# multigrid101/Opt

Measured on AMD Instinct MI355X. Metric: PCG JᵀJ·p throughput (unknowns/s) + GN iters/s, image_warping 4096² fp32, higher is better.
Workload: dtype f32; 1 GPU; image_warping 4096x4096 fp32 GN+PCG, lIterations=10; unknowns=50331648, parallelism=single

## Files before the change

opt_amd/csrc/common.h:

```cpp
#pragma once
#include <hip/hip_runtime.h>
#include <cstdio>
#include <cstdlib>
#include <cstdint>

#define OPT_HIP_CHECK(call)                                                         \
    do {                                                                            \
        hipError_t e_ = (call);                                                     \
        if (e_ != hipSuccess) {                                                     \
            fprintf(stderr, "[opt_amd] HIP error %d (%s) in %s at %s:%d\n", (int)e_,\
                    hipGetErrorString(e_), #call, __FILE__, __LINE__);              \
            exit(1);                                                                \
        }                                                                           \
    } while (0)

namespace optamd {

#define OPTAMD_HAVE_KBLOCK
constexpr int kWave = 64;
constexpr int kBlock = 256;
constexpr int kMaxReduce = 4;

struct Domain {
    int W, H;
    int y_lo, y_hi;
    int y_mem0, mem_rows;
    int edges = 0;
    __host__ __device__ long long npix_mem() const { return (long long)W * mem_rows; }
    __host__ __device__ long long off(int x, int yg) const {
        return (long long)(yg - y_mem0) * W + x;
    }
};

struct VecLayout {
    int nimg;
    int ch[4];
    long long off[5];
    long long N;
    long long fbase[4];
    __host__ __device__ static long long div_ch(long long l, int c) {
        switch (c) {
            case 1: return l;
            case 2: return l >> 1;
            case 3: return l < (1LL << 32) ? (long long)((unsigned)l / 3u) : l / 3;
            case 4: return l >> 2;
            default: return l / c;
        }
    }
    __host__ __device__ long long locate(long long e, int* img, long long* local) const {
        int k = 0;
        while (k + 1 < nimg && e >= off[k + 1]) ++k;
        *img = k;
        *local = e - off[k];
        return fbase[k] + div_ch(*local, ch[k]);
// ... 99 lines not shown
```

opt_amd/csrc/image_warping.hip:

```cpp
#include <hip/hip_runtime.h>
#include <hip/hip_ext.h>
#include <algorithm>
#include <type_traits>
#include <cmath>
#include <cstring>
#include <string>
#include "plan.h"
#include "pcg_kernels.h"
#include "stencil_plan.h"

namespace optamd {
namespace iw {
#pragma clang fp contract(on)

constexpr int kStrip = 64;

inline int rows_for(int nstrips, int nrows) {
    int rows = 32;
    while (rows > 16 && (long long)nstrips * ((nrows + 4 * rows - 1) / (4 * rows)) < 2048) rows /= 2;
    return rows;
}
inline int rows_one_round(int ngroups, int nrows, int ncu) {
    const long long slots = 4LL * 4 * ncu;
    for (int r = 8; r < 16; ++r)
        if ((long long)ngroups * ((nrows + r - 1) / r) * 4 <= slots) return r;
    return 16;
}

template <typename T>
struct Args {
    Domain dom;
    const T* O;
    const T* A;
    const float* U;
    const float* C;
    const float* M;
    uint8_t* flags;
    T wf, wr;
    int use_pre;
    int nstrips, nrowblocks, rows;
    int tb0, tn0, tb1;
    int side;
    int rev;
    T* S;
    T preO[2][5];
};

__shared__ float iw_ptab_f[16];
__shared__ double iw_ptab_d[16];
template <typename T> __device__ __forceinline__ T* iw_ptab();
template <> __device__ __forceinline__ float* iw_ptab<float>() { return iw_ptab_f; }
template <> __device__ __forceinline__ double* iw_ptab<double>() { return iw_ptab_d; }

template <typename T>
__device__ __forceinline__ T pre_offset(const Args<T>&, int f) {
    return (f & 1) ? iw_ptab<T>()[(f >> 1) & 15] : (T)0;
}
template <typename T>
__device__ __forceinline__ T pre_entry(const Args<T>& a, int k) {
    return k < 10 ? a.preO[k & 1][k >> 1] : (T)0;
}
#define IW_PRE_TABLE(a)                                                           \
    if (threadIdx.x < 16) iw_ptab<T>()[threadIdx.x] = pre_entry(a, threadIdx.x); \
    __syncthreads();

template <bool NT, typename T>
__device__ __forceinline__ T ld_v(const T* p) {
    if constexpr (NT) return __builtin_nontemporal_load(p);
    else return *p;
}
template <bool NT, typename T>
__device__ __forceinline__ void st_v(T* p, T v) {
    if constexpr (NT) __builtin_nontemporal_store(v, p);
    else *p = v;
}

// ... 42 lines not shown
__device__ __forceinline__ bool present(const Domain& d, int x, int y) {
    return x >= 0 && x < d.W && y >= 0 && y < d.H && y >= d.y_mem0 && y < d.y_mem0 + d.mem_rows;
}

template <typename T>
__device__ __forceinline__ void jedge(T pjx, T pjy, T pjt, T cj, T sj, float ujx, float ujy,
                                      T ptx, T pty, float utx, float uty, bool v, T wr,
                                      T& Jx, T& Jy, T& ax, T& ay) {
    const T dx = (T)(ujx - utx), dy = (T)(ujy - uty);
    ax = -sj * dx - cj * dy;
    ay = cj * dx - sj * dy;
    Jx = v ? wr * (pjx - ptx - ax * pjt) : (T)0;
    Jy = v ? wr * (pjy - pty - ay * pjt) : (T)0;
}

template <typename T>
__device__ __forceinline__ void eedge(T ojx, T ojy, T cj, T sj, float ujx, float ujy, T otx,
                                      T oty, float utx, float uty, bool v, T wr, T& ex, T& ey,
                                      T& ax, T& ay) {
    const T dx = (T)(ujx - utx), dy = (T)(ujy - uty);
    const T rx = cj * dx - sj * dy, ry = sj * dx + cj * dy;
    ax = -sj * dx - cj * dy;
    ay = cj * dx - sj * dy;
    ex = v ? wr * (ojx - otx - rx) : (T)0;
    ey = v ? wr * (ojy - oty - ry) : (T)0;
}

template <typename T>
__device__ __forceinline__ T diag_a2(T cj, T sj, float ujx, float ujy, float utx, float uty, T wr2) {
    const T dx = (T)(ujx - utx), dy = (T)(ujy - uty);
    const T ax = fmad(-sj, dx, -opaque(cj * dy));
    const T ay = fmad(cj, dx, -opaque(sj * dy));
    return opaque(wr2 * fmad(ax, ax, opaque(ay * ay)));
}

template <typename T>
__device__ __forceinline__ T pre_angle(T dt) {
    const T st = (T)1 + sqrt(dt);
    return (T)1 / (st * st);
}

typedef double acc_t;
template <typename T>
__device__ __forceinline__ T pcg_alpha(double rz, double pap) {
    return pap > 0.0 ? (T)(rz / pap) : (T)0;
}
template <typename T>
__device__ __forceinline__ acc_t dot3(T a0, T b0, T a1, T b1, T a2, T b2) {
    return (double)a0 * (double)b0 + (double)a1 * (double)b1 + (double)a2 * (double)b2;
}
template <typename T>
__device__ __forceinline__ acc_t wdot3(T w0, T a0, T b0, T w1, T a1, T b1, T w2, T a2, T b2) {
    (void)w1;
    return (double)w0 * ((double)a0 * (double)b0 + (double)a1 * (double)b1) + (double)w2 * ((double)a2 * (double)b2);
}

template <typename T>
struct PRaw {
    T v0, v1, v2;
    T w0, w1, w2;
    T q0, q1, q2;
    T d0, d1, d2;
    T ang;
    float2 u;
    int f, in;
    T ev0, ev1, ev2, ew0, ew1, ew2, eq0, eq1, eq2, eang;
// ... 480 lines not shown
                rapd += wdot3(cur.w0, cur.rx, aox, cur.w0, cur.ry, aoy, cur.w2, cur.rt, aot);
                apapd += wdot3(cur.w0, aox, aox, cur.w0, aoy, aoy, cur.w2, aot, aot);
            }
            in_up_x = jpy_x; in_up_y = jpy_y;
            my_x = jdn_x; my_y = jdn_y;
            thm = -wr * (adn_x * jdn_x + adn_y * jdn_y);
        };
        for (int y = g.y0; y < g.y1; y += 2) {
            const RRaw<T> n1 = raw(min(y + 2, g.y1));
            apply_row(A, B, y);
            A = fin(n1, y + 2);
            if (y + 1 >= g.y1) break;
            const RRaw<T> n2 = raw(min(y + 3, g.y1));
            apply_row(B, A, y + 1);
            B = fin(n2, y + 3);
        }
    }
    double v[4] = {(double)rzd, (double)papd, (double)rapd, (double)apapd};
    block_reduce_publish<4>(v, rs, g.tile);
}

template <typename T>
__device__ __forceinline__ vec2_t<T> shl2(vec2_t<T> v) {
    vec2_t<T> o;
    o.x = from_left0(v.x); o.y = from_left0(v.y);
    return o;
}
template <typename T>
__device__ __forceinline__ vec2_t<T> shr2(vec2_t<T> v) {
    vec2_t<T> o;
    o.x = from_right0(v.x); o.y = from_right0(v.y);
    return o;
}
template <typename T>
__device__ __forceinline__ void jedge2(vec2_t<T> pj, T pjt, T cj, T sj, vec2_t<float> uj, vec2_t<T> pt,
                                       vec2_t<float> ut, bool v, T wr, vec2_t<T>& J, vec2_t<T>& ad) {
    const vec2_t<float> du = uj - ut;
    const T dx = (T)du.x, dy = (T)du.y;
    vec2_t<T> ms, cs;
    ms.x = -sj; ms.y = cj;
    cs.x = cj; cs.y = sj;
    ad = ms * dx - cs * dy;
    const vec2_t<T> j = wr * ((pj - pt) - ad * pjt);
    J = v ? j : (vec2_t<T>)0;
}
template <typename T>
struct ACarry {
    vec2_t<T> in_up, my;
    T thm;
};
template <typename T>
__device__ __forceinline__ ACarry<T> acarry_init(vec2_t<T> up, T upt, T uc, T us, vec2_t<float> uu, bool uact,
                                                 vec2_t<T> cp, T cpt, T cc, T cs, vec2_t<float> cu, bool cact, T wr) {
    ACarry<T> k;
    vec2_t<T> ad;
    jedge2(up, upt, uc, us, uu, cp, cu, uact && cact, wr, k.in_up, ad);
    jedge2(cp, cpt, cc, cs, cu, up, uu, uact && cact, wr, k.my, ad);
    const vec2_t<T> th = ad * k.my;
    k.thm = -wr * (th.x + th.y);
    return k;
}
template <typename T>
__device__ __forceinline__ void apply_ap2(vec2_t<T> cp, T cpt, T cc, T cs, vec2_t<float> cu, bool cact, bool cfit,
                                          vec2_t<T> dp, T dpt, T dc, T ds, vec2_t<float> du, bool dact, T wr, T wf2,
                                          ACarry<T>& k, vec2_t<T>& ao, T& aot) {
    const vec2_t<T> lp = shl2(cp), rp = shr2(cp);
    const vec2_t<float> lu = shl2(cu), ru = shr2(cu);
    const int lact = from_left0_i((int)cact), ract = from_right0_i((int)cact);
    vec2_t<T> jpx, apx, jmx, amx, jpy, apy, jdn, adn;
    jedge2(cp, cpt, cc, cs, cu, rp, ru, cact && ract, wr, jpx, apx);
    jedge2(cp, cpt, cc, cs, cu, lp, lu, cact && lact, wr, jmx, amx);
    jedge2(cp, cpt, cc, cs, cu, dp, du, cact && dact, wr, jpy, apy);
    jedge2(dp, dpt, dc, ds, du, cp, cu, cact && dact, wr, jdn, adn);
    const vec2_t<T> inpx = shr2(jmx), inmx = shl2(jpx);
    ao = wr * ((jpx + jmx + jpy + k.my) - (inpx + inmx + jdn + k.in_up));
    if (cfit) ao += wf2 * cp;
    const vec2_t<T> tt = apx * jpx + amx * jmx + apy * jpy;
    aot = k.thm - wr * (tt.x + tt.y);
    if (!cact) { ao = (vec2_t<T>)0; aot = 0; }
    k.in_up = jpy;
    k.my = jdn;
    const vec2_t<T> th = adn * jdn;
    k.thm = -wr * (th.x + th.y);
}
typedef unsigned u32x2 __attribute__((ext_vector_type(2)));
typedef unsigned u32x4 __attribute__((ext_vector_type(4)));
__device__ __forceinline__ __amdgpu_buffer_rsrc_t bres(const void* p, unsigned bytes) {
    return __builtin_amdgcn_make_buffer_rsrc(const_cast<void*>(p), 0, p ? (int)bytes : 0, 0x00020000);
}
__device__ __forceinline__ void bst(__amdgpu_buffer_rsrc_t r, unsigned off, float v) {
    __builtin_amdgcn_raw_buffer_store_b32(__builtin_bit_cast(unsigned, v), r, off, 0, 0);
}
__device__ __forceinline__ void bst(__amdgpu_buffer_rsrc_t r, unsigned off, vec2_t<float> v) {
    __builtin_amdgcn_raw_buffer_store_b64(__builtin_bit_cast(u32x2, v), r, off, 0, 0);
}
__device__ __forceinline__ void bst(__amdgpu_buffer_rsrc_t r, unsigned off, double v) {
    __builtin_amdgcn_raw_buffer_store_b64(__builtin_bit_cast(u32x2, v), r, off, 0, 0);
}
__device__ __forceinline__ void bst(__amdgpu_buffer_rsrc_t r, unsigned off, vec2_t<double> v) {
    __builtin_amdgcn_raw_buffer_store_b128(__builtin_bit_cast(u32x4, v), r, off, 0, 0);
}
template <typename V> __device__ __forceinline__ V bld(__amdgpu_buffer_rsrc_t r, unsigned off);
template <> __device__ __forceinline__ float bld<float>(__amdgpu_buffer_rsrc_t r, unsigned off) {
    return __builtin_bit_cast(float, __builtin_amdgcn_raw_buffer_load_b32(r, off, 0, 0));
}
template <> __device__ __forceinline__ vec2_t<float> bld<vec2_t<float>>(__amdgpu_buffer_rsrc_t r, unsigned off) {
    return __builtin_bit_cast(vec2_t<float>, __builtin_amdgcn_raw_buffer_load_b64(r, off, 0, 0));
}
template <> __device__ __forceinline__ double bld<double>(__amdgpu_buffer_rsrc_t r, unsigned off) {
    return __builtin_bit_cast(double, __builtin_amdgcn_raw_buffer_load_b64(r, off, 0, 0));
}
template <> __device__ __forceinline__ vec2_t<double> bld<vec2_t<double>>(__amdgpu_buffer_rsrc_t r, unsigned off) {
    return __builtin_bit_cast(vec2_t<double>, __builtin_amdgcn_raw_buffer_load_b128(r, off, 0, 0));
}

template <typename T>
struct GRow {
    vec2_t<T> p;
    T pt;
    T c, s;
    vec2_t<float> u;
    int f;
    vec2_t<T> r;
    T rt, w2;
    vec2_t<T> d, q2;
    T dt, q2t;
    __device__ __forceinline__ bool act() const { return f & 1; }
    __device__ __forceinline__ bool fit() const { return (f >> 1) & 1; }
};
template <typename T>
struct GRaw {
    vec2_t<T> p, r, d, q2;
    T pt, rt, w2, ang, dt, q2t;
    vec2_t<float> u;
    int f, in;
};
template <typename T, int DM, int E, bool P0, bool REC, bool PRC = false>
__device__ __forceinline__ GRaw<T> raw_grow(const Args<T>& a, const WaveGeom& g, int y, unsigned tb, const T* pin,
                                            const T* rin, const T* pre, __amdgpu_buffer_rsrc_t rdl,
                                            __amdgpu_buffer_rsrc_t rq2, unsigned oob, bool own) {
    GRaw<T> q;
    q.in = present(a.dom, g.x, y);
    const unsigned i = q.in ? (unsigned)a.dom.off(g.x, y) : 0u;
    const POff<T> o(i, tb);
    q.f = ldb<false, uint8_t>(a.flags, i);
    own = own && g.out_lane;
    const unsigned oxy = own ? o.xy : oob, ot = own ? o.t : oob;
    if constexpr (REC) {
        const ROff<T> ro(i);
        ld_srec(a.S, ro.s, q.u, q.ang, q.w2);
        q.r = ldb<false, vec2_t<T>>(rin, ro.r);
        const vec2_t<T> tt = ldb<false, vec2_t<T>>(rin, ro.t);
        q.rt = tt.x; q.pt = tt.y;
        if (!(P0 && !E)) q.p = ldb<false, vec2_t<T>>(rin, ro.p);
        if (DM == 2) { q.d = bld<vec2_t<T>>(rdl, oxy); q.dt = bld<T>(rdl, ot); }
        if (E) {
            q.q2 = bld<vec2_t<T>>(rq2, own ? (P0 ? ro.r : ro.p) : oob);
            const vec2_t<T> t2 = bld<vec2_t<T>>(rq2, own ? ro.t : oob);
            q.q2t = P0 ? t2.x : t2.y;
        }
        return q;
    }
    q.u = ldb<false, vec2_t<float>>(a.U, 8u * i);
    q.ang = ldb<false, T>(a.A, o.s);
    q.r = ldb<false, vec2_t<T>>(rin, o.xy); q.rt = ldb<false, T>(rin, o.t);
    if constexpr (!PRC) q.w2 = ldb<false, T>(pre, o.s);
    else q.w2 = 0;
    if (!(P0 && !E)) { q.p = ldb<false, vec2_t<T>>(pin, o.xy); q.pt = ldb<false, T>(pin, o.t); }
    if (DM == 2) { q.d = bld<vec2_t<T>>(rdl, oxy); q.dt = bld<T>(rdl, ot); }
    if (E) { q.q2 = bld<vec2_t<T>>(rq2, oxy); q.q2t = bld<T>(rq2, ot); }
    return q;
}
template <typename T, int E, bool P0>
__device__ __forceinline__ GRow<T> finish_grow(const Args<T>& a, const GRaw<T>& q) {
    GRow<T> o;
    o.f = q.in ? q.f : 0;
    o.u = q.in ? q.u : (vec2_t<float>)0.f;
    sc_of(q.in ? q.ang : (T)0, &o.c, &o.s);
    o.r = q.r; o.rt = q.rt; o.w2 = q.w2;
    o.d = q.d; o.dt = q.dt;
    o.q2 = q.q2; o.q2t = q.q2t;
    if constexpr (P0) {
        const T w0 = pre_offset(a, o.f);
        if (E == 0) { o.p = opaque(w0 * q.r); o.pt = opaque(q.w2 * q.rt); }
        else { o.q2 = opaque(w0 * q.q2); o.q2t = opaque(q.w2 * q.q2t); o.p = q.p; o.pt = q.pt; }
    } else {
        o.p = q.p; o.pt = q.pt;
    }
    if (!o.act()) { o.p = (vec2_t<T>)0; o.pt = 0; }
    return o;
}
template <typename T>
struct HRow {
    vec2_t<T> p;
    T pt, c, s;
    vec2_t<float> u;
    bool act, fit;
    vec2_t<T> r;
    T rt, w0, w2;
};
template <typename T, int DM, int E, bool P0, bool U2, bool REC, bool PRC = false>
__device__ __forceinline__ void iw_pcg_body(const Args<T>& a, const T* __restrict__ pin, const T* __restrict__ rin,
                                            const T* __restrict__ pre, T* __restrict__ pout, T* rout,
                                            T* __restrict__ delta, double* __restrict__ sc, int prev,
                                            double base_scale, ReduceSlot rs, const T* pin2) {
    IW_PRE_TABLE(a);
    const WaveGeom g = geom_fused(a);
    const double rzp = sc[prev], papp = sc[prev + 1];
    const T alpha = pcg_alpha<T>(rzp, papp);
    const double alpha_d = (double)alpha;
    const double rz_id = base_scale * rzp - 2.0 * alpha_d * sc[prev + 2] + alpha_d * alpha_d * sc[prev + 3];
    const T beta = rz_id > 0.0 && rzp > 0.0 ? (T)(rz_id / rzp) : (T)0;
    const T alpha2 = E ? pcg_alpha<T>(sc[prev - kSlots], sc[prev - kSlots + 1]) : (T)0;
    if (blockIdx.x == 0 && threadIdx.x == 0) sc[prev + kSlots + 4] = rz_id;
    const T wr = a.wr, wf2 = a.wf * a.wf;
    const long long nplane = a.dom.npix_mem();
    const unsigned tb = (unsigned)(2 * nplane * (long long)sizeof(T));
    const unsigned vb = (unsigned)(3 * nplane * (long long)sizeof(T));
    const unsigned oob = REC ? 2u * vb : vb;
    const __amdgpu_buffer_rsrc_t r_out = bres(rout, oob), r_p = bres(pout, oob), r_d = bres(delta, vb),
                                 r_q2 = bres(pin2, oob);
    acc_t rzd = 0, papd = 0, rapd = 0, apapd = 0;
    if (g.y0 < g.y1) {
        auto raw = [&](int y) {
            return raw_grow<T, DM, E, P0, REC, PRC>(a, g, y, tb, pin, rin, pre, r_d, r_q2, oob, y >= g.y0 && y < g.y1);
        };
        auto fin = [&](const GRaw<T>& q) { return finish_grow<T, E, P0>(a, q); };
        ACarry<T> ka;
        const T wr2 = a.wr * a.wr;
        T dthm_a = 0;
        auto stage_a = [&](const GRow<T>& cur, const GRow<T>& dn, int y) {
            vec2_t<T> ap;
            T at;
            apply_ap2(cur.p, cur.pt, cur.c, cur.s, cur.u, cur.act(), cur.fit(), dn.p, dn.pt, dn.c, dn.s, dn.u,
                      dn.act(), wr, wf2, ka, ap, at);
            HRow<T> h;
            h.c = cur.c; h.s = cur.s; h.u = cur.u; h.act = cur.act(); h.fit = cur.fit();
            const T w0 = pre_offset(a, cur.f);
            h.r = cur.r - alpha * ap;
            h.rt = cur.rt - alpha * at;
            h.w0 = a.use_pre ? w0 : (T)1;
            if constexpr (PRC) {
                const vec2_t<float> lu = shl2(cur.u), ru = shr2(cur.u);
                const bool ca = cur.act(), da = dn.act();
                const bool lact = from_left0_i((int)ca) != 0, ract = from_right0_i((int)ca) != 0;
                const T dt = dthm_a + (ca && ract ? diag_a2(cur.c, cur.s, cur.u.x, cur.u.y, ru.x, ru.y, wr2) : (T)0) +
                             (ca && lact ? diag_a2(cur.c, cur.s, cur.u.x, cur.u.y, lu.x, lu.y, wr2) : (T)0) +
                             (ca && da ? diag_a2(cur.c, cur.s, cur.u.x, cur.u.y, dn.u.x, dn.u.y, wr2) : (T)0);
                dthm_a = ca && da ? diag_a2(dn.c, dn.s, dn.u.x, dn.u.y, cur.u.x, cur.u.y, wr2) : (T)0;
                h.w2 = a.use_pre ? (ca ? pre_angle(dt) : (T)0) : (T)1;
            } else {
                h.w2 = a.use_pre ? cur.w2 : (T)1;
            }
            const vec2_t<T> z = h.w0 * h.r;
            const T zt = h.w2 * h.rt;
            h.p = z + beta * cur.p;
            h.pt = zt + beta * cur.pt;
            const bool mine = y >= g.y0 && y < g.y1 && g.out_lane;
            {
                const unsigned iy = mine ? (unsigned)a.dom.off(g.x, y) : 0u;
                const POff<T> off(iy, tb);
                const unsigned oxy = mine ? off.xy : oob, ot = mine ? off.t : oob;
                if (DM != 0) {
                    vec2_t<T> d;
                    T dt;
                    if (E) {
                        if (DM == 1) { d = alpha2 * cur.q2; dt = alpha2 * cur.q2t; }
                        else { d = __builtin_elementwise_fma((vec2_t<T>)alpha2, cur.q2, cur.d); dt = fmad(alpha2, cur.q2t, cur.dt); }
                        d = __builtin_elementwise_fma((vec2_t<T>)alpha, cur.p, d); dt = fmad(alpha, cur.pt, dt);
                    } else if (DM == 1) {
                        d = alpha * cur.p; dt = alpha * cur.pt;
                    } else {
                        d = __builtin_elementwise_fma((vec2_t<T>)alpha, cur.p, cur.d); dt = fmad(alpha, cur.pt, cur.dt);
                    }
                    if (!h.act) { d = (vec2_t<T>)0; dt = 0; }
                    bst(r_d, oxy, d); bst(r_d, ot, dt);
                }
                if constexpr (REC) {
                    const ROff<T> ro(iy);
                    const vec2_t<T> pm = h.act ? h.p : (vec2_t<T>)0;
                    vec2_t<T> tt;
                    tt.x = h.rt; tt.y = h.act ? h.pt : (T)0;
                    bst(r_out, mine ? ro.r : oob, h.r); bst(r_out, mine ? ro.p : oob, pm);
                    bst(r_out, mine ? ro.t : oob, tt);
                } else {
                    bst(r_out, oxy, h.r); bst(r_out, ot, h.rt);
                }
                const acc_t rz = wdot3(h.w0, h.r.x, h.r.x, h.w0, h.r.y, h.r.y, h.w2, h.rt, h.rt);
                rzd += mine ? rz : 0.0;
            }
            if (!h.act) { h.p = (vec2_t<T>)0; h.pt = 0; }
            return h;
        };
        const int n = g.y1 - g.y0;
        const GRow<T> g0 = fin(raw(g.y0 - 2));
        GRow<T> qc = fin(raw(g.y0 - 1));
        GRow<T> qd = fin(raw(g.y0));
        ka = acarry_init(g0.p, g0.pt, g0.c, g0.s, g0.u, g0.act(), qc.p, qc.pt, qc.c, qc.s, qc.u, qc.act(), wr);
        if constexpr (PRC)
            dthm_a = g0.act() && qc.act() ? diag_a2(qc.c, qc.s, qc.u.x, qc.u.y, g0.u.x, g0.u.y, wr2) : (T)0;
        HRow<T> hup = stage_a(qc, qd, g.y0 - 1);
        qc = qd;
        qd = fin(raw(g.y0 + 1));
        HRow<T> hc = stage_a(qc, qd, g.y0);
        qc = qd;
        qd = fin(raw(g.y0 + 2));
        ACarry<T> kb = acarry_init(hup.p, hup.pt, hup.c, hup.s, hup.u, hup.act, hc.p, hc.pt, hc.c, hc.s, hc.u, hc.act, wr);
        auto stage_b = [&](const HRow<T>& cur, const HRow<T>& dn, int y) {
            vec2_t<T> ao;
            T aot;
            apply_ap2(cur.p, cur.pt, cur.c, cur.s, cur.u, cur.act, cur.fit, dn.p, dn.pt, dn.c, dn.s, dn.u, dn.act, wr,
                      wf2, kb, ao, aot);
            {
                if constexpr (!REC) {
                    const unsigned iy = g.out_lane ? (unsigned)a.dom.off(g.x, y) : 0u;
                    const POff<T> off(iy, tb);
                    bst(r_p, g.out_lane ? off.xy : oob, cur.p); bst(r_p, g.out_lane ? off.t : oob, cur.pt);
                }
                const acc_t s1 = dot3(cur.p.x, ao.x, cur.p.y, ao.y, cur.pt, aot);
                const acc_t s2 = wdot3(cur.w0, cur.r.x, ao.x, cur.w0, cur.r.y, ao.y, cur.w2, cur.rt, aot);
                const acc_t s3 = wdot3(cur.w0, ao.x, ao.x, cur.w0, ao.y, ao.y, cur.w2, aot, aot);
                papd += g.out_lane ? s1 : 0.0;
                rapd += g.out_lane ? s2 : 0.0;
                apapd += g.out_lane ? s3 : 0.0;
            }
        };
        if constexpr (!U2) {
            for (int k = 0; k < n; ++k) {
                const GRaw<T> nx = raw(g.y0 + min(k + 3, n + 1));
                const HRow<T> hd = stage_a(qc, qd, g.y0 + k + 1);
                stage_b(hc, hd, g.y0 + k);
                hc = hd;
                qc = qd;
                qd = fin(nx);
            }
        } else {
            GRow<T> q0 = qc, q1 = qd;
            HRow<T> h0 = hc, h1;
            for (int k = 0; k < n; k += 2) {
                const GRaw<T> n1 = raw(g.y0 + min(k + 3, n + 1));
                h1 = stage_a(q0, q1, g.y0 + k + 1);
                stage_b(h0, h1, g.y0 + k);
                q0 = fin(n1);
                if (k + 1 >= n) break;
                const GRaw<T> n2 = raw(g.y0 + min(k + 4, n + 1));
                h0 = stage_a(q1, q0, g.y0 + k + 2);
                stage_b(h1, h0, g.y0 + k + 1);
                q1 = fin(n2);
            }
        }
    }
    double v[4] = {(double)rzd, (double)papd, (double)rapd, (double)apapd};
    block_reduce_publish<4>(v, rs, g.tile);
}
template <typename T, int DM, int E = 0, bool P0 = false, bool U2 = false, bool REC = false, bool PRC = false>
__global__ __launch_bounds__(kBlock) void iw_pcg(Args<T> a, const T* __restrict__ pin, const T* __restrict__ rin,
                                                 const T* __restrict__ pre, T* __restrict__ pout, T* rout,
                                                 T* __restrict__ delta, double* __restrict__ sc, int prev,
                                                 double base_scale, ReduceSlot rs, const T* pin2 = nullptr) {
    iw_pcg_body<T, DM, E, P0, U2, REC, PRC>(a, pin, rin, pre, pout, rout, delta, sc, prev, base_scale, rs, pin2);
}

template <typename T>
struct VRaw {
    Vec2<T> o;
    T t;
    float2 u, c;
    float m;
    int in;
    Vec2<T> eo;
    T et;
    float2 eu;
    float em;
    int ein;
};
template <typename T>
struct VRow {
    T ox, oy, t, c, s;
    float ux, uy, cx, cy;
    int act, fit;
    T eox, eoy;
    float eux, euy;
    int eact;
    T ec, es;
};
template <typename T, bool EDGE_ANGLE, bool EDGE = true>
__device__ __forceinline__ VRaw<T> raw_vrow(const Args<T>& a, const WaveGeom& g, int y) {
    VRaw<T> q;
    q.in = present(a.dom, g.x, y);
    if (!EDGE) {
        const unsigned i = q.in ? (unsigned)a.dom.off(g.x, y) : 0u;
        const vec2_t<T> o = ldb<false, vec2_t<T>>(a.O, i * 2u * (unsigned)sizeof(T));
        q.o = Vec2<T>{o.x, o.y};
// ... 820 lines not shown
        for (int k = 0; k < 2 && k < max_images; ++k) {
            if (offset) offset[k] = k * 2 * N;
            if (elements) elements[k] = N;
            if (channels) channels[k] = ch[k];
        }
        return 2;
    }
    std::string family() const override { return "image_warping"; }
    std::string apply_kernel_name() const override { return "iw_apply"; }

    void init(void** params) override {
        begin_call();
        bind(params, true);
        exchange_unknowns();
        tbegin("iw_cost"); launch_cost(kScCost); tend();
        allreduce(kScCost);
        prev_cost_ = read_scalar(kScCost);
        n_iter_ = 0;
        initialised_ = true;
        end_call();
        if (opts_.verbosity > 0) fprintf(stderr, "[opt_amd] init cost %.9g\n", prev_cost_);
    }

    int step(void** params) override {
        if (!initialised_) init(params);
        if (n_iter_ >= sp_.nIterations) {
            cleanup_log();
            return 0;
        }
        begin_call();
        bind(params, false);
        exchange_unknowns();
        const int L = std::max(0, sp_.lIterations);
        red_.ensure(std::max({stencil_blocks(), fused_blocks(), fused_side_blocks(), kUpdBlocks}), 4,
                    kScBase + iw::kSlots * (L + 2));
        T* pcur = p0_;
        T* pprev = p1_;
        const bool fused = fused_init_ && offsets32_ && L >= 1;
        const bool res = fused_res_ && offsets32_ && L >= 1;
        const bool allp = allp_ && fused_init_ && offsets32_ && res && apfree_ && !recl_ && L >= 2 &&
                          L <= iw::kAllPMax && ensure_pall(L);
        const bool defer = res && defer_ && !allp;
        T* pb[3] = {p0_, p1_, p2_};
        const bool keep0 = allp && res && L >= 3;
        if (allp) pcur = pall_;
        const bool p0 = res && L >= 3;
        const bool apfree = res && apfree_;
        const bool rec = recl_ && fused && apfree;
        if (rec) { pcur = rec_[0]; pb[0] = rec_[0]; pb[1] = rec_[1]; pb[2] = rec_[2]; }
        if (fused) {
            launch_jtf_apply(p0 ? nullptr : pcur, L == 1 || apfree, rec);
            allreduce(rz(0), 4);
            if (distributed()) {
                std::vector<HaloPlane> pl;
                if (rec) {
                    pl.push_back({(void*)rec_[0], 6 * sizeof(T) * dom_.W});
                    pl.push_back({(void*)srec_, 4 * sizeof(T) * dom_.W});
                } else {
                    add_vec_planes(pl, r_);
                    pl.push_back({(void*)pre_, sizeof(T) * dom_.W});
                    if (!p0) add_vec_planes(pl, pcur);
                    if (!apfree) add_vec_planes(pl, Ap_);
                }
                pl.push_back({(void*)flags_, (size_t)dom_.W});
                exchange(pl);
            }
        } else {
            tbegin("iw_jtf"); launch_jtf(r_, pre_, rz(0), false, res); tend();
// ... 183 lines not shown
        begin_call();
        bind(params, false);
        launch_flags();
        hipEvent_t e0, e1;
        OPT_HIP_CHECK(hipEventCreate(&e0));
        OPT_HIP_CHECK(hipEventCreate(&e1));
        launch_apply<0, 0>((const T*)p, nullptr, kScTmp, 0, 0, 0, 0, (T*)Ap);
        OPT_HIP_CHECK(hipEventRecord(e0, stream_));
        for (int i = 0; i < reps; ++i) launch_apply<0, 0>((const T*)p, nullptr, kScTmp, 0, 0, 0, 0, (T*)Ap);
        OPT_HIP_CHECK(hipEventRecord(e1, stream_));
        OPT_HIP_CHECK(hipEventSynchronize(e1));
        float ms = 0;
        OPT_HIP_CHECK(hipEventElapsedTime(&ms, e0, e1));
        (void)hipEventDestroy(e0);
        (void)hipEventDestroy(e1);
        end_call();
        return 1000.0 * ms / std::max(1, reps);
    }

private:
    void read_knobs() {
        const int rw = env_int("OPT_AMD_ROWS", 0);
        if (rw > 0) { rows_ = rw; rows_auto_ = false; }
        fused_init_ = env_int("OPT_AMD_IW_FUSED_INIT", 1) != 0;
        fused_res_ = env_int("OPT_AMD_IW_FUSED_RES", 1) != 0;
        defer_ = env_int("OPT_AMD_IW_DEFER", 1) != 0;
        apfree_ = env_int("OPT_AMD_IW_APFREE", 1) != 0;
        rec_on_ = env_int("OPT_AMD_IW_REC", 0) != 0;
        allp_ = env_int("OPT_AMD_IW_ALLP", 1) != 0;
        pcg_u2_ = env_int("OPT_AMD_IW_PCG_U2", 1) != 0;
        pall_limit_mb_ = env_int("OPT_AMD_IW_ALLP_LIMIT_MB", -1);
        upd_pairs_ = env_int("OPT_AMD_IW_UPD_PAIRS", 1) != 0;
        pcg_prc_ = env_int("OPT_AMD_IW_PCG_PRC", 1) != 0;
        cost_flags_ = env_int("OPT_AMD_IW_COST_FLAGS", 1) != 0;
        mall_rev_ = env_int("OPT_AMD_IW_MALL_REV", 1) != 0;
    }
    static constexpr size_t kSlack = 1 << 20;
    static constexpr size_t kStagger = 36864;
    static constexpr int kUpdBlocks = 2048;
    void* vec_alloc(size_t bytes) {
        char* p = (char*)dmalloc(bytes + kSlack);
        raw_.push_back(p);
        OPT_HIP_CHECK(hipMemset(p, 0, bytes + kSlack));
        return p;
    }
    void place() {
        T** vs[] = {&r_, &p0_, &p1_, &Ap_, &delta_, &r1_, &Ap1_, &pre_, &p2_};
        if (raw_.size() < 10) return;
        for (int k = 0; k < 8; ++k) *vs[k] = (T*)(raw_[k] + (kStagger * k) % kSlack);
        flags_ = (uint8_t*)(raw_[8] + (kStagger * 8) % kSlack);
        p2_ = (T*)(raw_[9] + (kStagger * 9) % kSlack);
        if (recl_ && raw_.size() >= 14) {
            for (int k = 0; k < 3; ++k) rec_[k] = (T*)(raw_[10 + k] + (kStagger * (10 + k)) % kSlack);
            srec_ = (T*)(raw_[13] + (kStagger * 13) % kSlack);
        }
    }
    void allocate() {
        const long long N = dom_.npix_mem();
        nvec_ = 3 * N;
        offsets32_ = iw::offsets_fit_32<T>(N);
        for (T** v : {&r_, &p0_, &p1_, &Ap_, &delta_, &r1_, &Ap1_})
            *v = (T*)vec_alloc(sizeof(T) * 3 * N);
        pre_ = (T*)vec_alloc(sizeof(T) * N);
        flags_ = (uint8_t*)vec_alloc(N);
        p2_ = (T*)vec_alloc(sizeof(T) * 3 * N);
        recl_ = rec_on_ && fused_init_ && fused_res_ && apfree_ && iw::offsets_fit_rec<T>(N);
// ... 89 lines not shown
        raw_.clear();
        dfree(pall_);
        pall_ = nullptr;
        pall_cap_ = 0;
        for (T** v : {&r_, &pre_, &p0_, &p1_, &Ap_, &delta_, &r1_, &Ap1_, &p2_}) *v = nullptr;
        flags_ = nullptr;
        for (T*& v : rec_) v = nullptr;
        srec_ = nullptr;
        for (T** v : {&dO_, &dA_}) { dfree(*v); *v = nullptr; }
        for (float** v : {&dU_, &dC_, &dM_}) { dfree(*v); *v = nullptr; }
    }

    bool distributed() const { return comm_ && comm_->size() > 1; }
    void allreduce(int idx, int n = 1) {
        if (distributed()) comm_->allreduce_sum(red_.scalars + idx, n, stream_);
    }
    void add_vec_planes(std::vector<HaloPlane>& v, const T* x) const {
        const long long plane = dom_.npix_mem();
        v.push_back({(void*)x, sizeof(T) * 2 * dom_.W});
        v.push_back({(void*)(x + 2 * plane), sizeof(T) * dom_.W});
    }
    void exchange(const std::vector<HaloPlane>& planes) {
        if (!distributed()) return;
        tbegin("halo_exchange");
        comm_->halo_exchange(planes, dom_, halo(), stream_);
        tend();
    }
    void exchange_unknowns() {
        exchange({{(void*)cur_O_, sizeof(T) * 2 * dom_.W}, {(void*)cur_A_, sizeof(T) * dom_.W}});
    }

    static constexpr int kScCost = 0, kScTmp = 1, kScBase = 2;
    int rz(int i) const { return kScBase + iw::kSlots * i; }
    int pap(int i) const { return rz(i) + 1; }

    int stencil_blocks() const { return nstrips_ * nrowblocks_; }
    int fused_strips() const { return (dom_.W + iw::kFStrip - 1) / iw::kFStrip; }
    int side_chunks() const { return (dom_.y_hi - dom_.y_lo + rows_ - 1) / rows_; }
    int fused_side_blocks() const {
        return (fused_strips() + kBlock / kWave - 1) / (kBlock / kWave) * side_chunks();
    }
    int fused_blocks() const { return fused_strips() * nrowblocks_; }

    iw::Args<T> args() const {
        iw::Args<T> a;
        a.dom = dom_;
        a.O = cur_O_; a.A = cur_A_; a.U = cur_U_; a.C = cur_C_; a.M = cur_M_;
        a.flags = flags_;
        a.wf = (T)wf_; a.wr = (T)wr_;
        a.use_pre = spec_.use_preconditioner ? 1 : 0;
        a.nstrips = nstrips_; a.nrowblocks = nrowblocks_; a.rows = rows_;
        a.tb0 = 0; a.tn0 = nstrips_ * nrowblocks_; a.tb1 = 0;
        a.side = 0;
        a.rev = 0;
        a.S = srec_;
        const T wr2 = (T)wr_ * (T)wr_, wf2 = (T)wf_ * (T)wf_;
        for (int fit = 0; fit < 2; ++fit)
            for (int nv = 0; nv < 5; ++nv) {
                T d = wr2 * (T)(2 * nv);
                if (fit) d += wf2;
                const T s1 = (T)1 + std::sqrt(d);
                a.preO[fit][nv] = spec_.use_preconditioner ? (T)1 / (s1 * s1) : (T)0.25;
            }
        return a;
    }

    void bind(void** params, bool ) {
        wf_ = *(const float*)params[idx_wf_];
        wr_ = *(const float*)params[idx_wr_];
        user_O_ = (T*)params[idx_O_];
        user_A_ = (T*)params[idx_A_];
        if (!opts_.host_buffers) {
            cur_O_ = user_O_; cur_A_ = user_A_;
            cur_U_ = (const float*)params[idx_U_];
            cur_C_ = (const float*)params[idx_C_];
            cur_M_ = (const float*)params[idx_M_];
        } else {
            const long long N = dom_.npix_mem();
            OPT_HIP_CHECK(hipMemcpyAsync(dO_, user_O_, sizeof(T) * 2 * N, hipMemcpyHostToDevice, stream_));
            OPT_HIP_CHECK(hipMemcpyAsync(dA_, user_A_, sizeof(T) * N, hipMemcpyHostToDevice, stream_));
            OPT_HIP_CHECK(hipMemcpyAsync(dU_, params[idx_U_], sizeof(float) * 2 * N, hipMemcpyHostToDevice, stream_));
            OPT_HIP_CHECK(hipMemcpyAsync(dC_, params[idx_C_], sizeof(float) * 2 * N, hipMemcpyHostToDevice, stream_));
            OPT_HIP_CHECK(hipMemcpyAsync(dM_, params[idx_M_], sizeof(float) * N, hipMemcpyHostToDevice, stream_));
            cur_O_ = dO_; cur_A_ = dA_; cur_U_ = dU_; cur_C_ = dC_; cur_M_ = dM_;
        }
    }
    void unbind_after_step() {
// ... 35 lines not shown
        a.nstrips = fused_strips();
        const int nb = fused_blocks();
        a.tb0 = 0; a.tn0 = nb; a.tb1 = 0;
        if (rec) {
            if (!no_ap || (pout && pout != rec_[0])) throw std::logic_error("iw_jtf_apply<REC>: record 0 only, no Ap");
            launch_timed("iw_jtf_apply", iw::iw_jtf_apply<T, true>, nb, a, rec_[0], (T*)nullptr, pout, (T*)nullptr,
                         red_.slot(nb, rz(0)));
            return;
        }
        launch_timed("iw_jtf_apply", iw::iw_jtf_apply<T>, nb, a, r_, pre_, pout,
                     no_ap ? nullptr : Ap_, red_.slot(nb, rz(0)));
    }
    void launch_pcg(int i, const T* pin, T* pout, bool last, const T* pin2, bool p0, int part = 0, bool rec = false,
                    bool nodelta = false, bool keep0 = false) {
        const T* rin = rec ? pin : rvec(i - 1, keep0);
        T* rout = rec ? pout : (last ? nullptr : rvec(i, keep0));
        const double base_scale = (i == 1 && !spec_.use_preconditioner) ? 4.0 : 1.0;
        iw::Args<T> a = args();
        const int fs = fused_strips();
        a.nstrips = fs;
        const int ng = (fs + kBlock / kWave - 1) / (kBlock / kWave), nch = side_chunks();
        const int nb = ng * nch;
        a.side = 1;
        a.tb0 = 0; a.tn0 = nb; a.tb1 = 0;
        int grid = nb;
        if (part == 1) {
            a.tb0 = ng; a.tn0 = ng * (nch - 2);
            grid = a.tn0;
        } else if (part == 2) {
            a.tb0 = 0; a.tn0 = ng; a.tb1 = ng * (nch - 1);
            grid = 2 * ng;
        }
        a.rev = mall_rev_ && (i & 1) ? 1 : 0;
        const ReduceSlot rs = red_.slot(nb, rz(i));
        auto go = [&](auto kern) {
            launch_timed("iw_pcg", kern, grid, a, pin, rin, (const T*)pre_, pout, rout, delta_, red_.scalars,
                         rz(i - 1), base_scale, rs, pin2);
        };
        auto pick = [&](auto u2, auto dp) {
            constexpr bool U2 = decltype(u2)::value, DP = decltype(dp)::value;
            if (nodelta) {
                if (i == 1 && p0) go(iw::iw_pcg<T, 0, 0, true, U2, DP>);
                else if (pcg_prc_ && !DP) go(iw::iw_pcg<T, 0, 0, false, U2, false, true>);
                else go(iw::iw_pcg<T, 0, 0, false, U2, DP>);
            } else if (pin2 || (defer_ && i == 1)) {
                if (i == 1 && p0) go(iw::iw_pcg<T, 0, 0, true, U2, DP>);
                else if (i % 2 == 1) go(iw::iw_pcg<T, 0, 0, false, U2, DP>);
                else if (i == 2 && p0) go(iw::iw_pcg<T, 1, 1, true, U2, DP>);
                else if (i == 2) go(iw::iw_pcg<T, 1, 1, false, U2, DP>);
                else go(iw::iw_pcg<T, 2, 1, false, U2, DP>);
            } else if (i == 1 && p0) go(iw::iw_pcg<T, 1, 0, true, U2, DP>);
            else if (i == 1) go(iw::iw_pcg<T, 1, 0, false, U2, DP>);
            else go(iw::iw_pcg<T, 2, 0, false, U2, DP>);
        };
        using F = std::false_type;
        using Tt = std::true_type;
        if (rec) pick(F{}, Tt{});
        else if (rows_ >= 16 && pcg_u2_) pick(Tt{}, F{});
        else pick(F{}, F{});
    }
    template <int MODE, int DM>
    void launch_apply(const T* pin, T* pout, int sc_out, int ib_num, int ib_den, int ia_num, int ia_den,
                      T* Ap = nullptr, bool no_ap = false, int part = 0, bool sums = false) {
        const int nb = stencil_blocks();
        Ap = no_ap ? nullptr : (Ap ? Ap : Ap_);
        iw::Args<T> a = args();
        int grid = nb;
        if (part == 1) {
            a.tb0 = nstrips_; a.tn0 = nstrips_ * (nrowblocks_ - 2);
            grid = a.tn0;
        } else if (part == 2) {
            a.tb0 = 0; a.tn0 = nstrips_; a.tb1 = nstrips_ * (nrowblocks_ - 1);
            grid = 2 * nstrips_;
        }
// ... 68 lines not shown
                hipLaunchKernelGGL(iw::iw_cost60<T>, dim3(nb), dim3(kBlock), 0, stream_, a, red_.slot(nb, sc_out));
        } else {
            const int nb = stencil_blocks();
            hipLaunchKernelGGL(iw::iw_cost<T>, dim3(nb), dim3(kBlock), 0, stream_, args(), red_.slot(nb, sc_out));
        }
        OPT_HIP_CHECK(hipGetLastError());
    }
    void launch_flags() {
        hipLaunchKernelGGL(iw::iw_flags<T>, dim3(flat_grid(dom_.npix_mem(), 1)), dim3(kBlock), 0, stream_,
                           args());
        OPT_HIP_CHECK(hipGetLastError());
    }

    Domain dom_;
    int idx_O_, idx_A_, idx_U_, idx_C_, idx_M_, idx_wf_, idx_wr_;
    long long nvec_ = 0;
    T *r_ = nullptr, *pre_ = nullptr, *p0_ = nullptr, *p1_ = nullptr, *Ap_ = nullptr, *delta_ = nullptr;
    T *r1_ = nullptr, *Ap1_ = nullptr;
    T* p2_ = nullptr;
    std::vector<char*> raw_;
    uint8_t* flags_ = nullptr;
    bool fused_init_ = true;
    bool fused_res_ = true;
    bool defer_ = true;
    bool apfree_ = true;
    bool rec_on_ = false;
    bool allp_ = true;
    T* pall_ = nullptr;
    int pall_cap_ = 0;
    bool pall_warned_ = false;
    bool mall_rev_ = true;
    bool cost_flags_ = true;
    bool pcg_prc_ = true;
    bool upd_pairs_ = true;
    long long pall_limit_mb_ = -1;
    bool recl_ = false;
    T* rec_[3] = {nullptr, nullptr, nullptr};
    T* srec_ = nullptr;
    bool pcg_u2_ = true;
    bool offsets32_ = true;
    int rows_ = 0, nstrips_ = 0, nrowblocks_ = 0;
    bool rows_auto_ = true;
    Comm* comm_ = nullptr;
    const bool overlap_ = env_int("OPT_AMD_HALO_OVERLAP", 1) != 0;
    float wf_ = 0, wr_ = 0;
    T *user_O_ = nullptr, *user_A_ = nullptr;
    T *cur_O_ = nullptr, *cur_A_ = nullptr;
    const float *cur_U_ = nullptr, *cur_C_ = nullptr, *cur_M_ = nullptr;
    T *dO_ = nullptr, *dA_ = nullptr;
    float *dU_ = nullptr, *dC_ = nullptr, *dM_ = nullptr;
};

template <typename TT>
class ImageWarpingOp {
public:
    using T = TT;
    static constexpr const char* kName = "image_warping";
    static constexpr const char* kApplyName = "iw_apply";
    static constexpr bool kSlabs = true;
    ImageWarpingOp(const ProblemSpec& spec, const StateOptions& opts, Domain dom) : dom_(dom), opts_(opts) {
        idx_O_ = spec.unknown(0)->index;
        idx_A_ = spec.unknown(1)->index;
        idx_U_ = spec.array(0)->index;
        idx_C_ = spec.array(1)->index;
        idx_M_ = spec.array(2)->index;
        std::vector<DeclParam> ps = spec.params;
// ... 131 lines not shown
```

Before: 170.0 billion unknowns/s.

## Add wave-uniform fast path for fully active rows in fused PCG kernel

Adds a specialised path in the fused image-warping PCG kernel for rows where the whole wavefront is active. That path skips the per-lane activity masking and DPP neighbour-activity shuffles, and stage B reuses edge angle derivatives that stage A already computed. It also adds an optional deeper row-prefetch variant (off by default) and a fast-row counter reduced as a fifth reduction slot. In exchange there is more ballot work per row, a larger reduction payload, extra register pressure from carrying the edge terms, and more template instantiations.

```diff
diff --git a/opt_amd/csrc/common.h b/opt_amd/csrc/common.h
--- a/opt_amd/csrc/common.h
+++ b/opt_amd/csrc/common.h
@@ -19,7 +19,7 @@
 #define OPTAMD_HAVE_KBLOCK
 constexpr int kWave = 64;
 constexpr int kBlock = 256;
-constexpr int kMaxReduce = 4;
+constexpr int kMaxReduce = 5;
 
 struct Domain {
     int W, H;
diff --git a/opt_amd/csrc/image_warping.hip b/opt_amd/csrc/image_warping.hip
--- a/opt_amd/csrc/image_warping.hip
+++ b/opt_amd/csrc/image_warping.hip
@@ -42,6 +42,7 @@
     int tb0, tn0, tb1;
     int side;
     int rev;
+    int fast;
     T* S;
     T preO[2][5];
 };
@@ -150,6 +151,11 @@
     const T ax = fmad(-sj, dx, -opaque(cj * dy));
     const T ay = fmad(cj, dx, -opaque(sj * dy));
     return opaque(wr2 * fmad(ax, ax, opaque(ay * ay)));
+}
+
+template <typename T, typename V>
+__device__ __forceinline__ T diag_a2_ad(V ad, T wr2) {
+    return opaque(wr2 * fmad(ad.x, ad.x, opaque(ad.y * ad.y)));
 }
 
 template <typename T>
@@ -696,7 +702,7 @@
     o.x = from_right0(v.x); o.y = from_right0(v.y);
     return o;
 }
-template <typename T>
+template <typename T, bool F = false>
 __device__ __forceinline__ void jedge2(vec2_t<T> pj, T pjt, T cj, T sj, vec2_t<float> uj, vec2_t<T> pt,
                                        vec2_t<float> ut, bool v, T wr, vec2_t<T>& J, vec2_t<T>& ad) {
     const vec2_t<float> du = uj - ut;
@@ -706,8 +712,20 @@
     cs.x = cj; cs.y = sj;
     ad = ms * dx - cs * dy;
     const vec2_t<T> j = wr * ((pj - pt) - ad * pjt);
-    J = v ? j : (vec2_t<T>)0;
-}
+    if constexpr (F) J = opaque(j);
+    else J = v ? j : (vec2_t<T>)0;
+}
+template <typename T, bool F = false>
+__device__ __forceinline__ void jedge2_ad(vec2_t<T> pj, T pjt, vec2_t<T> pt, vec2_t<T> ad, bool v, T wr,
+                                          vec2_t<T>& J) {
+    const vec2_t<T> j = wr * ((pj - pt) - ad * pjt);
+    if constexpr (F) J = opaque(j);
+    else J = v ? j : (vec2_t<T>)0;
+}
+template <typename T>
+struct EdgeAd {
+    vec2_t<T> px, mx, py, dn;
+};
 template <typename T>
 struct ACarry {
     vec2_t<T> in_up, my;
@@ -724,24 +742,42 @@
     k.thm = -wr * (th.x + th.y);
     return k;
 }
-template <typename T>
+template <typename T, bool F = false, bool AD = false>
 __device__ __forceinline__ void apply_ap2(vec2_t<T> cp, T cpt, T cc, T cs, vec2_t<float> cu, bool cact, bool cfit,
                                           vec2_t<T> dp, T dpt, T dc, T ds, vec2_t<float> du, bool dact, T wr, T wf2,
-                                          ACarry<T>& k, vec2_t<T>& ao, T& aot) {
+                                          ACarry<T>& k, vec2_t<T>& ao, T& aot, bool anyfit = true,
+                                          EdgeAd<T>* ead = nullptr) {
     const vec2_t<T> lp = shl2(cp), rp = shr2(cp);
-    const vec2_t<float> lu = shl2(cu), ru = shr2(cu);
-    const int lact = from_left0_i((int)cact), ract = from_right0_i((int)cact);
+    bool vpx = true, vmx = true, vy = true;
+    if constexpr (!F) {
+        const int lact = from_left0_i((int)cact), ract = from_right0_i((int)cact);
+        vpx = cact && ract; vmx = cact && lact; vy = cact && dact;
+    }
     vec2_t<T> jpx, apx, jmx, amx, jpy, apy, jdn, adn;
-    jedge2(cp, cpt, cc, cs, cu, rp, ru, cact && ract, wr, jpx, apx);
-    jedge2(cp, cpt, cc, cs, cu, lp, lu, cact && lact, wr, jmx, amx);
-    jedge2(cp, cpt, cc, cs, cu, dp, du, cact && dact, wr, jpy, apy);
-    jedge2(dp, dpt, dc, ds, du, cp, cu, cact && dact, wr, jdn, adn);
+    if constexpr (AD) {
+        apx = ead->px; amx = ead->mx; apy = ead->py; adn = ead->dn;
+        jedge2_ad<T, F>(cp, cpt, rp, apx, vpx, wr, jpx);
+        jedge2_ad<T, F>(cp, cpt, lp, amx, vmx, wr, jmx);
+        jedge2_ad<T, F>(cp, cpt, dp, apy, vy, wr, jpy);
+        jedge2_ad<T, F>(dp, dpt, cp, adn, vy, wr, jdn);
+    } else {
+        const vec2_t<float> lu = shl2(cu), ru = shr2(cu);
+        jedge2<T, F>(cp, cpt, cc, cs, cu, rp, ru, vpx, wr, jpx, apx);
+        jedge2<T, F>(cp, cpt, cc, cs, cu, lp, lu, vmx, wr, jmx, amx);
+        jedge2<T, F>(cp, cpt, cc, cs, cu, dp, du, vy, wr, jpy, apy);
+        jedge2<T, F>(dp, dpt, dc, ds, du, cp, cu, vy, wr, jdn, adn);
+        if (ead) { ead->px = apx; ead->mx = amx; ead->py = apy; ead->dn = adn; }
+    }
     const vec2_t<T> inpx = shr2(jmx), inmx = shl2(jpx);
     ao = wr * ((jpx + jmx + jpy + k.my) - (inpx + inmx + jdn + k.in_up));
-    if (cfit) ao += wf2 * cp;
+    if (!F || anyfit) {
+        if (cfit) ao += wf2 * cp;
+    }
     const vec2_t<T> tt = apx * jpx + amx * jmx + apy * jpy;
     aot = k.thm - wr * (tt.x + tt.y);
-    if (!cact) { ao = (vec2_t<T>)0; aot = 0; }
+    if constexpr (!F) {
+        if (!cact) { ao = (vec2_t<T>)0; aot = 0; }
+    }
     k.in_up = jpy;
     k.my = jdn;
     const vec2_t<T> th = adn * jdn;
@@ -789,6 +825,7 @@
     T rt, w2;
     vec2_t<T> d, q2;
     T dt, q2t;
+    bool full, anyfit;
     __device__ __forceinline__ bool act() const { return f & 1; }
     __device__ __forceinline__ bool fit() const { return (f >> 1) & 1; }
 };
@@ -835,10 +872,12 @@
     if (E) { q.q2 = bld<vec2_t<T>>(rq2, oxy); q.q2t = bld<T>(rq2, ot); }
     return q;
 }
-template <typename T, int E, bool P0>
+template <typename T, int E, bool P0, bool CLS>
 __device__ __forceinline__ GRow<T> finish_grow(const Args<T>& a, const GRaw<T>& q) {
     GRow<T> o;
     o.f = q.in ? q.f : 0;
+    o.full = CLS && a.fast && __builtin_amdgcn_ballot_w64(o.act()) == ~0ull;
+    o.anyfit = __builtin_amdgcn_ballot_w64(o.fit()) != 0ull;
     o.u = q.in ? q.u : (vec2_t<float>)0.f;
     sc_of(q.in ? q.ang : (T)0, &o.c, &o.s);
     o.r = q.r; o.rt = q.rt; o.w2 = q.w2;
@@ -860,14 +899,16 @@
     T pt, c, s;
     vec2_t<float> u;
     bool act, fit;
+    bool full, anyfit;
     vec2_t<T> r;
     T rt, w0, w2;
+    EdgeAd<T> ead;
 };
-template <typename T, int DM, int E, bool P0, bool U2, bool REC, bool PRC = false>
+template <typename T, int DM, int E, bool P0, bool U2, bool REC, bool PRC = false, bool PF2 = false>
 __device__ __forceinline__ void iw_pcg_body(const Args<T>& a, const T* __restrict__ pin, const T* __restrict__ rin,
                                             const T* __restrict__ pre, T* __restrict__ pout, T* rout,
                                             T* __restrict__ delta, double* __restrict__ sc, int prev,
-                                            double base_scale, ReduceSlot rs, const T* pin2) {
+                                            double base_scale, ReduceSlot rs, const T* pin2, double* nfast_out) {
     IW_PRE_TABLE(a);
     const WaveGeom g = geom_fused(a);
     const double rzp = sc[prev], papp = sc[prev + 1];
@@ -876,7 +917,6 @@
     const double rz_id = base_scale * rzp - 2.0 * alpha_d * sc[prev + 2] + alpha_d * alpha_d * sc[prev + 3];
     const T beta = rz_id > 0.0 && rzp > 0.0 ? (T)(rz_id / rzp) : (T)0;
     const T alpha2 = E ? pcg_alpha<T>(sc[prev - kSlots], sc[prev - kSlots + 1]) : (T)0;
-    if (blockIdx.x == 0 && threadIdx.x == 0) sc[prev + kSlots + 4] = rz_id;
     const T wr = a.wr, wf2 = a.wf * a.wf;
     const long long nplane = a.dom.npix_mem();
     const unsigned tb = (unsigned)(2 * nplane * (long long)sizeof(T));
@@ -885,26 +925,34 @@
     const __amdgpu_buffer_rsrc_t r_out = bres(rout, oob), r_p = bres(pout, oob), r_d = bres(delta, vb),
                                  r_q2 = bres(pin2, oob);
     acc_t rzd = 0, papd = 0, rapd = 0, apapd = 0;
+    int nfast = 0;
     if (g.y0 < g.y1) {
         auto raw = [&](int y) {
             return raw_grow<T, DM, E, P0, REC, PRC>(a, g, y, tb, pin, rin, pre, r_d, r_q2, oob, y >= g.y0 && y < g.y1);
         };
-        auto fin = [&](const GRaw<T>& q) { return finish_grow<T, E, P0>(a, q); };
+        constexpr bool CLS = U2 && (sizeof(T) == 4 || DM == 0), CAR = U2 && sizeof(T) == 4;
+        auto fin = [&](const GRaw<T>& q) { return finish_grow<T, E, P0, CLS>(a, q); };
         ACarry<T> ka;
         const T wr2 = a.wr * a.wr;
         T dthm_a = 0;
-        auto stage_a = [&](const GRow<T>& cur, const GRow<T>& dn, int y) {
+        auto stage_a = [&](auto ft, const GRow<T>& cur, const GRow<T>& dn, int y) {
+            constexpr bool F = decltype(ft)::value;
             vec2_t<T> ap;
             T at;
-            apply_ap2(cur.p, cur.pt, cur.c, cur.s, cur.u, cur.act(), cur.fit(), dn.p, dn.pt, dn.c, dn.s, dn.u,
-                      dn.act(), wr, wf2, ka, ap, at);
             HRow<T> h;
+            apply_ap2<T, F>(cur.p, cur.pt, cur.c, cur.s, cur.u, cur.act(), cur.fit(), dn.p, dn.pt, dn.c, dn.s, dn.u,
+                            dn.act(), wr, wf2, ka, ap, at, cur.anyfit, &h.ead);
             h.c = cur.c; h.s = cur.s; h.u = cur.u; h.act = cur.act(); h.fit = cur.fit();
-            const T w0 = pre_offset(a, cur.f);
+            h.full = cur.full; h.anyfit = cur.anyfit;
+            const T w0 = F ? iw_ptab<T>()[(cur.f >> 1) & 15] : pre_offset(a, cur.f);
             h.r = cur.r - alpha * ap;
             h.rt = cur.rt - alpha * at;
             h.w0 = a.use_pre ? w0 : (T)1;
-            if constexpr (PRC) {
+            if constexpr (PRC && F) {
+                const T dt = dthm_a + diag_a2_ad(h.ead.px, wr2) + diag_a2_ad(h.ead.mx, wr2) + diag_a2_ad(h.ead.py, wr2);
+                dthm_a = diag_a2_ad(h.ead.dn, wr2);
+                h.w2 = a.use_pre ? pre_angle(dt) : (T)1;
+            } else if constexpr (PRC) {
                 const vec2_t<float> lu = shl2(cur.u), ru = shr2(cur.u);
                 const bool ca = cur.act(), da = dn.act();
                 const bool lact = from_left0_i((int)ca) != 0, ract = from_right0_i((int)ca) != 0;
@@ -937,7 +985,9 @@
                     } else {
                         d = __builtin_elementwise_fma((vec2_t<T>)alpha, cur.p, cur.d); dt = fmad(alpha, cur.pt, cur.dt);
                     }
-                    if (!h.act) { d = (vec2_t<T>)0; dt = 0; }
+                    if constexpr (!F) {
+                        if (!h.act) { d = (vec2_t<T>)0; dt = 0; }
+                    }
                     bst(r_d, oxy, d); bst(r_d, ot, dt);
                 }
                 if constexpr (REC) {
@@ -953,7 +1003,11 @@
                 const acc_t rz = wdot3(h.w0, h.r.x, h.r.x, h.w0, h.r.y, h.r.y, h.w2, h.rt, h.rt);
                 rzd += mine ? rz : 0.0;
             }
-            if (!h.act) { h.p = (vec2_t<T>)0; h.pt = 0; }
+            if constexpr (F) {
+                h.p = opaque(h.p); h.pt = opaque(h.pt);
+            } else {
+                if (!h.act) { h.p = (vec2_t<T>)0; h.pt = 0; }
+            }
             return h;
         };
         const int n = g.y1 - g.y0;
@@ -963,18 +1017,21 @@
         ka = acarry_init(g0.p, g0.pt, g0.c, g0.s, g0.u, g0.act(), qc.p, qc.pt, qc.c, qc.s, qc.u, qc.act(), wr);
         if constexpr (PRC)
             dthm_a = g0.act() && qc.act() ? diag_a2(qc.c, qc.s, qc.u.x, qc.u.y, g0.u.x, g0.u.y, wr2) : (T)0;
-        HRow<T> hup = stage_a(qc, qd, g.y0 - 1);
+        using Ff = std::false_type;
+        using Ft = std::true_type;
+        HRow<T> hup = stage_a(Ff{}, qc, qd, g.y0 - 1);
         qc = qd;
         qd = fin(raw(g.y0 + 1));
-        HRow<T> hc = stage_a(qc, qd, g.y0);
+        HRow<T> hc = stage_a(Ff{}, qc, qd, g.y0);
         qc = qd;
         qd = fin(raw(g.y0 + 2));
         ACarry<T> kb = acarry_init(hup.p, hup.pt, hup.c, hup.s, hup.u, hup.act, hc.p, hc.pt, hc.c, hc.s, hc.u, hc.act, wr);
-        auto stage_b = [&](const HRow<T>& cur, const HRow<T>& dn, int y) {
+        auto stage_b = [&](auto ft, const HRow<T>& cur, const HRow<T>& dn, int y) {
             vec2_t<T> ao;
             T aot;
-            apply_ap2(cur.p, cur.pt, cur.c, cur.s, cur.u, cur.act, cur.fit, dn.p, dn.pt, dn.c, dn.s, dn.u, dn.act, wr,
-                      wf2, kb, ao, aot);
+            EdgeAd<T> ead = cur.ead;
+            apply_ap2<T, decltype(ft)::value, CAR>(cur.p, cur.pt, cur.c, cur.s, cur.u, cur.act, cur.fit, dn.p, dn.pt,
+                                                  dn.c, dn.s, dn.u, dn.act, wr, wf2, kb, ao, aot, cur.anyfit, &ead);
             {
                 if constexpr (!REC) {
                     const unsigned iy = g.out_lane ? (unsigned)a.dom.off(g.x, y) : 0u;
@@ -989,11 +1046,21 @@
                 apapd += g.out_lane ? s3 : 0.0;
             }
         };
+        auto step = [&](const GRow<T>& qa, const GRow<T>& qb, const HRow<T>& hb, HRow<T>& ha, int y) {
+            if (qa.full && qb.full && hb.full) {
+                ++nfast;
+                ha = stage_a(Ft{}, qa, qb, y + 1);
+                stage_b(Ft{}, hb, ha, y);
+            } else {
+                ha = stage_a(Ff{}, qa, qb, y + 1);
+                stage_b(Ff{}, hb, ha, y);
+            }
+        };
         if constexpr (!U2) {
             for (int k = 0; k < n; ++k) {
                 const GRaw<T> nx = raw(g.y0 + min(k + 3, n + 1));
-                const HRow<T> hd = stage_a(qc, qd, g.y0 + k + 1);
-                stage_b(hc, hd, g.y0 + k);
+                HRow<T> hd;
+                step(qc, qd, hc, hd, g.y0 + k);
                 hc = hd;
                 qc = qd;
                 qd = fin(nx);
@@ -1001,28 +1068,46 @@
         } else {
             GRow<T> q0 = qc, q1 = qd;
             HRow<T> h0 = hc, h1;
+            if constexpr (PF2) {
+                auto row = [&](int j) { return g.y0 + min(j, n + 1); };
+                GRaw<T> ra = raw(row(3)), rb;
+                for (int k = 0; k < n; k += 2) {
+                    rb = raw(row(k + 4));
+                    step(q0, q1, h0, h1, g.y0 + k);
+                    q0 = fin(ra);
+                    if (k + 1 >= n) break;
+                    ra = raw(row(k + 5));
+                    step(q1, q0, h1, h0, g.y0 + k + 1);
+                    q1 = fin(rb);
+                }
+            } else
             for (int k = 0; k < n; k += 2) {
                 const GRaw<T> n1 = raw(g.y0 + min(k + 3, n + 1));
-                h1 = stage_a(q0, q1, g.y0 + k + 1);
-                stage_b(h0, h1, g.y0 + k);
+                step(q0, q1, h0, h1, g.y0 + k);
                 q0 = fin(n1);
                 if (k + 1 >= n) break;
                 const GRaw<T> n2 = raw(g.y0 + min(k + 4, n + 1));
-                h0 = stage_a(q1, q0, g.y0 + k + 2);
-                stage_b(h1, h0, g.y0 + k + 1);
+                step(q1, q0, h1, h0, g.y0 + k + 1);
                 q1 = fin(n2);
             }
         }
     }
-    double v[4] = {(double)rzd, (double)papd, (double)rapd, (double)apapd};
-    block_reduce_publish<4>(v, rs, g.tile);
-}
-template <typename T, int DM, int E = 0, bool P0 = false, bool U2 = false, bool REC = false, bool PRC = false>
+    double v[5] = {(double)rzd, (double)papd, (double)rapd, (double)apapd, g.lane == 0 ? (double)nfast : 0.0};
+    double tot[5];
+    if (block_reduce_publish<5>(v, rs, g.tile, tot)) {
+        __hip_atomic_store(&rs.out[4], rz_id, __ATOMIC_RELAXED, __HIP_MEMORY_SCOPE_AGENT);
+        if (nfast_out) *nfast_out = tot[4];
+    }
+}
+template <typename T, int DM, int E = 0, bool P0 = false, bool U2 = false, bool REC = false, bool PRC = false,
+          bool PF2 = false>
 __global__ __launch_bounds__(kBlock) void iw_pcg(Args<T> a, const T* __restrict__ pin, const T* __restrict__ rin,
                                                  const T* __restrict__ pre, T* __restrict__ pout, T* rout,
                                                  T* __restrict__ delta, double* __restrict__ sc, int prev,
-                                                 double base_scale, ReduceSlot rs, const T* pin2 = nullptr) {
-    iw_pcg_body<T, DM, E, P0, U2, REC, PRC>(a, pin, rin, pre, pout, rout, delta, sc, prev, base_scale, rs, pin2);
+                                                 double base_scale, ReduceSlot rs, const T* pin2 = nullptr,
+                                                 double* nfast_out = nullptr) {
+    iw_pcg_body<T, DM, E, P0, U2, REC, PRC, PF2>(a, pin, rin, pre, pout, rout, delta, sc, prev, base_scale, rs, pin2,
+                                                 nfast_out);
 }
 
 template <typename T>
@@ -1909,8 +1994,8 @@
         bind(params, false);
         exchange_unknowns();
         const int L = std::max(0, sp_.lIterations);
-        red_.ensure(std::max({stencil_blocks(), fused_blocks(), fused_side_blocks(), kUpdBlocks}), 4,
-                    kScBase + iw::kSlots * (L + 2));
+        red_.ensure(std::max({stencil_blocks(), fused_blocks(), fused_side_blocks(), kUpdBlocks}), 5,
+                    kScBase + iw::kSlots * (L + 2) + L);
         T* pcur = p0_;
         T* pprev = p1_;
         const bool fused = fused_init_ && offsets32_ && L >= 1;
@@ -2160,6 +2245,8 @@
         pall_limit_mb_ = env_int("OPT_AMD_IW_ALLP_LIMIT_MB", -1);
         upd_pairs_ = env_int("OPT_AMD_IW_UPD_PAIRS", 1) != 0;
         pcg_prc_ = env_int("OPT_AMD_IW_PCG_PRC", 1) != 0;
+        pcg_fast_ = env_int("OPT_AMD_IW_PCG_FAST", 1) != 0;
+        pcg_pf_ = env_int("OPT_AMD_IW_PCG_PF", 1);
         cost_flags_ = env_int("OPT_AMD_IW_COST_FLAGS", 1) != 0;
         mall_rev_ = env_int("OPT_AMD_IW_MALL_REV", 1) != 0;
     }
@@ -2315,6 +2402,7 @@
 
     static constexpr int kScCost = 0, kScTmp = 1, kScBase = 2;
     int rz(int i) const { return kScBase + iw::kSlots * i; }
+    int nfast(int i) const { return kScBase + iw::kSlots * (std::max(0, sp_.lIterations) + 2) + i; }
     int pap(int i) const { return rz(i) + 1; }
 
     int stencil_blocks() const { return nstrips_ * nrowblocks_; }
@@ -2336,6 +2424,7 @@
         a.tb0 = 0; a.tn0 = nstrips_ * nrowblocks_; a.tb1 = 0;
         a.side = 0;
         a.rev = 0;
+        a.fast = 0;
         a.S = srec_;
         const T wr2 = (T)wr_ * (T)wr_, wf2 = (T)wf_ * (T)wf_;
         for (int fit = 0; fit < 2; ++fit)
@@ -2437,14 +2526,19 @@
             grid = 2 * ng;
         }
         a.rev = mall_rev_ && (i & 1) ? 1 : 0;
+        a.fast = pcg_fast_ ? 1 : 0;
         const ReduceSlot rs = red_.slot(nb, rz(i));
         auto go = [&](auto kern) {
             launch_timed("iw_pcg", kern, grid, a, pin, rin, (const T*)pre_, pout, rout, delta_, red_.scalars,
-                         rz(i - 1), base_scale, rs, pin2);
+                         rz(i - 1), base_scale, rs, pin2, red_.scalars + nfast(i));
         };
         auto pick = [&](auto u2, auto dp) {
             constexpr bool U2 = decltype(u2)::value, DP = decltype(dp)::value;
-            if (nodelta) {
+            if (nodelta && U2 && !DP && pcg_pf_ == 2) {
+                if (i == 1 && p0) go(iw::iw_pcg<T, 0, 0, true, U2, false, false, U2>);
+                else if (pcg_prc_) go(iw::iw_pcg<T, 0, 0, false, U2, false, true, U2>);
+                else go(iw::iw_pcg<T, 0, 0, false, U2, false, false, U2>);
+            } else if (nodelta) {
                 if (i == 1 && p0) go(iw::iw_pcg<T, 0, 0, true, U2, DP>);
                 else if (pcg_prc_ && !DP) go(iw::iw_pcg<T, 0, 0, false, U2, false, true>);
                 else go(iw::iw_pcg<T, 0, 0, false, U2, DP>);
@@ -2579,6 +2673,8 @@
     bool mall_rev_ = true;
     bool cost_flags_ = true;
     bool pcg_prc_ = true;
+    int pcg_pf_ = 1;
+    bool pcg_fast_ = true;
     bool upd_pairs_ = true;
     long long pall_limit_mb_ = -1;
     bool recl_ = false;
```

Measured after the change: 166.7 billion unknowns/s. -2.0%, worse.
